# cinemere/evacuation

Hardware: AMD Instinct MI355X
Metric: env-steps/s (agent-updates/s) at n=60x4096 envs (higher is better)
Workload: dtype f32

## Files before the change

evacuation_amd/csrc/evac_api.hip:

```cpp
#include <hip/hip_runtime.h>

#include <cmath>
#include <cstddef>
#include <cstdio>
#include <cstdlib>
#include <cstring>
#include <mutex>
#include <new>
#include <string>
#include <vector>

#include "evac_device.h"
#include "evac_subwave.h"
#include "evac_team.h"
#include "evac_gather.h"
#include "evac_policy.h"
#include "evac_host.h"

namespace {

thread_local std::string g_create_error;

int validate(const evac_config_t* c, std::string& err) {
    if (!c) { err = "cfg is NULL"; return EVAC_ERR_INVALID_ARGUMENT; }
// ... 8 lines not shown
    if (c->type != EVAC_TYPE_DICT && c->type != EVAC_TYPE_BOX) { err = "type must be Dict|Box"; return EVAC_ERR_INVALID_ARGUMENT; }
    if (c->positions == EVAC_POS_GRAV && c->type == EVAC_TYPE_BOX) {
        err = "positions='grav' with type='Box' is not implemented (reference wrappers/config.py:79-80 raises NotImplementedError)";
        return EVAC_ERR_UNSUPPORTED;
    }
    return EVAC_OK;
}

int64_t obs_dim_of(const evac_config_t* c) {
    const int64_t n = c->number_of_pedestrians;
    if (c->positions == EVAC_POS_GRAV) return 6;
    const int64_t sc = c->statuses == EVAC_STAT_OHE ? 4 : (c->statuses == EVAC_STAT_CAT ? 1 : 0);
    if (c->type == EVAC_TYPE_BOX) return (n + 2) * (2 + sc);
    return 4 + 2 * n + sc * n;
}

}

enum class Form { Plain, Parts, Chain, Persist };

struct evac_handle {
    evac_config_t cfg;
    evac::Params p;
    int device;
    bool bound;
    int sub_lanes;
    bool cells;
    bool cu_wide;
    bool cu_wide4;
    bool default_cfg;
    int team_k;
    int32_t* sched;
    int sched_gen = -1;
    bool team_bound;
    int team_fit = -1;
    size_t team_xchg_bytes;
    bool team_coop;
    int cus;
    bool team_fault;
    volatile unsigned* team_flag_host;
    unsigned* team_flag_dev;
    std::string err;
    std::string variant[4];
    evac_options_t opt;
    Form form = Form::Plain;
    struct OwnStreams {
        hipStream_t s[2];
        hipEvent_t done[2], fork;
        bool pending;
        bool forked;
    } own;
    evac_handle* part[2];
    char* xchg;
    size_t xchg_bytes;
    unsigned* abort_word;
    hipEvent_t last_ev;
    struct ChainState {
        bool bound;
        bool small;
        bool restart = true;
        bool dirty;
        int gen = 1;
        int start = 1;
        int32_t* sched;
        unsigned long long wgs;
    } chain;
// ... 436 lines not shown
    __atomic_thread_fence(__ATOMIC_SEQ_CST);
    c->seq = (unsigned)h->persist.seq + 1u;
    __atomic_thread_fence(__ATOMIC_SEQ_CST);
    h->persist.seq += 1;
}
void release_own(evac_handle* h) {
    DeviceGuard g(h->device);
    for (int k = 0; k < 2; ++k)
        if (h->own.s[k]) (void)hipStreamSynchronize(h->own.s[k]);
    if (h->own.s[0] && h->own.s[1] && pools_on()) {
        std::lock_guard<std::mutex> lk(g_pool_mu);
        g_pool_pairs.push_back(PooledPair{h->device, {h->own.s[0], h->own.s[1]}});
        h->own.s[0] = h->own.s[1] = nullptr;
    }
    for (int k = 0; k < 2; ++k) {
        if (h->own.s[k]) (void)hipStreamDestroy(h->own.s[k]);
        if (h->own.done[k]) (void)hipEventDestroy(h->own.done[k]);
        if (h->part[k]) {
            give_error_word(h->device, (void*)h->part[k]->team_flag_host, (void*)h->part[k]->team_flag_dev);
            delete h->part[k];
        }
        h->part[k] = nullptr;
    }
    if (h->own.fork) (void)hipEventDestroy(h->own.fork);
    if (h->last_ev) (void)hipEventDestroy(h->last_ev);
    give_uncached(h->device, h->xchg, h->xchg_bytes);
    h->own = {};
    h->xchg = nullptr;
    h->xchg_bytes = 0;
    h->last_ev = nullptr;
    h->form = Form::Plain;
}
void deal_now(evac_handle_t h, hipStream_t s, bool both);
struct Deal { const int32_t* perm; int32_t* moving; const int32_t* loads; int32_t* next; };
Deal deal_of(const evac_handle* h, bool deals) {
    const int E = h->p.n_envs, g = h->sched_gen;
    const bool dealt = h->sched && g >= 0;
    deals = deals && dealt;
    return Deal{dealt ? h->sched + (2 + (g & 1)) * E : nullptr, h->sched ? h->sched + (dealt ? (g & 1) : 0) * E : nullptr,
                deals ? h->sched + ((g + 1) & 1) * E : nullptr, deals ? h->sched + (2 + ((g + 1) & 1)) * E : nullptr};
}
int launch_persistent(evac_handle* h, int resume, int stop_at, bool fresh) {
    using FW = evac::Wave<1, 1024>;
    using FW4 = evac::Wave<4, 1024>;
    hipStream_t S = h->own.s[0];
    const int E = h->p.n_envs;
    if (h->sched && h->sched_gen < 0) deal_now(h, S, true);
    const Deal d = deal_of(h, fresh);
    if (d.next) h->sched_gen += 1;
    evac::ChainArgs ca{h->xchg, h->persist.seq, nullptr, nullptr, 0, nullptr, resume, stop_at};
    if (h->team_k) {
        int32_t* decision = (int32_t*)(h->xchg + (size_t)evac::kPersistRing * 64 + 128) + E;
        if (hipMemsetAsync(h->p.team_rec, 0xff, h->team_xchg_bytes, S) != hipSuccess || hipMemsetAsync(decision, 0, 4 * (size_t)E, S) != hipSuccess) {
            (void)hipGetLastError();
            return fail(h, EVAC_ERR_HIP, "evac_rollout (persistent team kernel): hipMemsetAsync failed");
        }
        const int* np_ = nullptr;
        int* nq_ = nullptr;
        void* argv[] = {(void*)&h->p, (void*)&np_, (void*)&nq_, (void*)&np_, (void*)&nq_, (void*)&ca};
        const hipError_t le = launch_team_grid(h, team_persist_kernel(h), argv, S, true, false);
        if (le != hipSuccess) return fail(h, EVAC_ERR_HIP, std::string("evac_rollout (persistent team kernel): ") + hipGetErrorString(le));
    } else {
        const bool four = h->cu_wide4;
        const auto fn = four ? EVAC_PICK(h, k_rollout_persist_default_config, k_rollout_persist, FW4)
                             : EVAC_PICK(h, k_rollout_persist_default_config, k_rollout_persist, FW);
        const dim3 grid((unsigned)(E / (four ? FW4::kEnvsPerBlock : FW::kEnvsPerBlock)));
        hipLaunchKernelGGL(fn, grid, dim3(four ? FW4::kBlock : FW::kBlock), 0, S, h->p, d.perm, d.moving, d.loads, d.next, ca);
    }
    if (const int lc = check_launch(h, "evac_rollout (persistent kernel)"); lc != EVAC_OK) return lc;
    if (hipEventRecord(h->last_ev, S) != hipSuccess) { (void)hipGetLastError(); return fail(h, EVAC_ERR_HIP, "evac_rollout: event record behind the persistent kernel failed"); }
    return EVAC_OK;
}
int stop_persistent(evac_handle* h) {
    const int stop_index = h->persist.seq;
    post_command(h, 0, nullptr, nullptr, nullptr);
    h->persist.running = false;
    return launch_persistent(h, 1, stop_index, false);
}
int settle(evac_handle* h, hipStream_t stream, bool host_wait = false) {
    if (h->form == Form::Chain) h->chain.restart = true;
    if (!h->own.pending) return EVAC_OK;
// ... 152 lines not shown
    return EVAC_OK;
}

int64_t evac_obs_dim(evac_handle_t h) { return h ? h->p.obs_dim : -1; }
int32_t evac_num_envs(evac_handle_t h) { return h ? h->p.n_envs : -1; }

int64_t evac_algorithmic_bytes_per_env_step(evac_handle_t h) {
    if (!h) return -1;
    return 32ll * h->p.n_ped + 38ll + 4ll * h->p.obs_dim;
}

int evac_bind_state(evac_handle_t h, float* ped, uint8_t* status, float* agent, int32_t* clock, float* acc) {
    if (!h) return EVAC_ERR_INVALID_ARGUMENT;
    if (!ped || !status || !agent || !clock || !acc) return fail(h, EVAC_ERR_INVALID_ARGUMENT, "evac_bind_state: NULL buffer");
    if (((uintptr_t)ped | (uintptr_t)agent | (uintptr_t)clock | (uintptr_t)acc) & 15u)
        return fail(h, EVAC_ERR_INVALID_ARGUMENT, "evac_bind_state: ped/agent/clock/acc must be 16-byte aligned");
    if (const int rc = settle(h, nullptr, true); rc != EVAC_OK) return rc;
    h->p.ped = (float4*)ped;
    h->p.status = status;
    h->p.agent = (float4*)agent;
    h->p.clock = (int4*)clock;
    h->p.acc = (float4*)acc;
    h->bound = true;
    for (int k = 0; k < (h->form == Form::Parts ? 2 : 0); ++k) {
        const size_t first = (size_t)k * (size_t)h->part[k]->p.n_envs, N = (size_t)h->p.n_ped;
        const int rc = evac_bind_state(h->part[k], ped + first * N * 4, status + first * N, agent + first * 4, clock + first * 4, acc + first * 4);
        if (rc != EVAC_OK) return fail(h, rc, std::string("evac_bind_state (part): ") + h->part[k]->err);
    }
    return EVAC_OK;
}

namespace {
struct WorkspaceLayout {
    size_t sched, stats, team_rec, team_tile, team_xchg_end, chain_sched, chain_abort, total;
};
WorkspaceLayout workspace_layout(const evac_handle* h) {
    const size_t E = (size_t)h->p.n_envs;
    auto up = [](size_t x) { return (x + 255) & ~(size_t)255; };
    WorkspaceLayout w{};
    size_t o = 0;
    w.sched = o; o = up(o + 4 * E * sizeof(int32_t));
    w.stats = o; o = up(o + 64);
    if (h->form == Form::Chain) {
        w.chain_sched = o; o = up(o + 8 * E * sizeof(int32_t));
        w.chain_abort = o; o = up(o + 128);
    }
    if (h->team_k) {
        w.team_rec = o; o = up(o + evac::kTeamSets * E * 32 * 16);
        w.team_tile = o; o = up(o + evac::kTeamSets * E * 1024 * 16);
        w.team_xchg_end = o;
    }
    w.total = o;
    return w;
}
}

int64_t evac_workspace_bytes(evac_handle_t h) {
    if (!h) return -1;
    size_t total = workspace_layout(h).total, parts = 0;
    for (int k = 0; k < (h->form == Form::Parts ? 2 : 0); ++k) parts += workspace_layout(h->part[k]).total;
    return (int64_t)(parts > total ? parts : total);
}

int evac_bind_workspace(evac_handle_t h, void* workspace, int64_t bytes) {
    if (!h) return EVAC_ERR_INVALID_ARGUMENT;
    if (const int rc = settle(h, nullptr, true); rc != EVAC_OK) return rc;
    h->sched = nullptr;
    h->sched_gen = -1;
    h->team_bound = false;
    h->chain.bound = false;
    if (h->form == Form::Parts) {
        if (workspace && (bytes < evac_workspace_bytes(h) || ((uintptr_t)workspace & 255u)))
            return fail(h, EVAC_ERR_INVALID_ARGUMENT, "evac_bind_workspace: workspace smaller than evac_workspace_bytes() or not 256-byte aligned");
        size_t o = 0;
        for (int k = 0; k < 2; ++k) {
            const size_t t = workspace_layout(h->part[k]).total;
            const int rc = evac_bind_workspace(h->part[k], workspace ? (char*)workspace + o : nullptr, (int64_t)t);
            if (rc != EVAC_OK) return fail(h, rc, std::string("evac_bind_workspace (part): ") + h->part[k]->err);
            o += t;
        }
        return EVAC_OK;
    }
    if (!workspace) return EVAC_OK;
    const WorkspaceLayout w = workspace_layout(h);
    if (bytes < (int64_t)w.total) return fail(h, EVAC_ERR_INVALID_ARGUMENT, "evac_bind_workspace: workspace smaller than evac_workspace_bytes()");
    if ((uintptr_t)workspace & 255u) return fail(h, EVAC_ERR_INVALID_ARGUMENT, "evac_bind_workspace: workspace must be 256-byte aligned");
    char* base = (char*)workspace;
    h->sched = (int32_t*)(base + w.sched);
    if (h->form == Form::Chain) {
        h->chain.sched = (int32_t*)(base + w.chain_sched);
        h->abort_word = (unsigned*)(base + w.chain_abort);
        h->chain.dirty = false;
        h->chain.wgs = 0;
        h->chain.bound = true;
    }
    if (h->team_k) {
        h->p.team_err = h->team_flag_dev;
        h->p.team_rec = base + w.team_rec;
        h->p.team_tile = base + w.team_tile;
        h->team_xchg_bytes = w.team_xchg_end - w.team_rec;
        h->team_bound = true;
        DeviceGuard g(h->device);
        (void)team_grid_fits(h);
    }
    return EVAC_OK;
}

namespace {
void deal_now(evac_handle_t h, hipStream_t s, bool both) {
    const int E = h->p.n_envs;
    if (h->sched_gen < 0) h->sched_gen = 0;
    const int g = h->sched_gen;
    hipLaunchKernelGGL(evac::k_schedule, dim3(1), dim3(1024), 0, s, E, (const int*)(h->sched + ((g + 1) & 1) * E),
                       h->sched + (2 + (g & 1)) * E, both ? h->sched + (2 + ((g + 1) & 1)) * E : (int32_t*)nullptr,
                       h->cu_wide4 ? 4 : 16, h->cu_wide4 ? 4 : 1, 0);
}
}

int evac_reschedule(evac_handle_t h, void* stream) {
    if (!h) return EVAC_ERR_INVALID_ARGUMENT;
    if (const int rc = settle(h, (hipStream_t)stream); rc != EVAC_OK) return rc;
    if (h->form == Form::Chain) return EVAC_OK;
    if (h->form == Form::Parts) {
        for (int k = 0; k < 2; ++k)
            if (const int rc = evac_reschedule(h->part[k], stream); rc != EVAC_OK) return fail(h, rc, h->part[k]->err);
        return EVAC_OK;
    }
    if (!h->sched || !(h->cu_wide || h->cu_wide4)) return EVAC_OK;
    DeviceGuard g(h->device);
    deal_now(h, (hipStream_t)stream, true);
    return check_launch(h, "evac_reschedule");
}

int32_t evac_schedule_generation(evac_handle_t h) {
    if (h && h->form == Form::Parts) return evac_schedule_generation(h->part[0]);
    return (h && h->sched && (h->cu_wide || h->cu_wide4)) ? h->sched_gen : -1;
}

int evac_peer_gather(const float* src, int64_t rows, int32_t row_words, int32_t take_words, float* const* peer_dst, int32_t world,
                     int32_t my_rank, int32_t wgs_per_peer, void* stream) {
    if (!src || !peer_dst || rows <= 0 || row_words <= 0 || take_words <= 0 || take_words > row_words || world < 1 ||
        world > evac::kMaxPeers || my_rank < 0 || my_rank >= world)
        return EVAC_ERR_INVALID_ARGUMENT;
    if (rows * (int64_t)take_words >= (int64_t)1 << 31) return EVAC_ERR_INVALID_ARGUMENT;
    evac::PeerPtrs pp{};
    for (int r = 0; r < world; ++r) {
        if (!peer_dst[r]) return EVAC_ERR_INVALID_ARGUMENT;
        pp.dst[r] = peer_dst[r];
// ... 137 lines not shown
        h->persist.first = h->persist.seq;
    } else if (hipEventQuery(h->last_ev) == hipSuccess) {
        if (const int rc = launch_persistent(h, 1, 0x7fffffff, false); rc != EVAC_OK) return rc;
    } else {
        (void)hipGetLastError();
    }
    post_command(h, (int)n_steps, slab_out, final_stats, nullptr);
    h->own.pending = true;
    return EVAC_OK;
}

static int rollout_chain(evac_handle* h, int32_t n_steps, const float* actions, float* slab_out, evac_episode_stats_t* final_stats, hipStream_t s_) {
    using FW = evac::Wave<1, 1024>;
    using FW4 = evac::Wave<4, 1024>;
    using FS = evac::Wave<1, 256>;
    evac_handle::ChainState& ch = h->chain;
    const int wpe = h->cu_wide4 ? 4 : 1, per_wg = (h->cu_wide4 || ch.small) ? 4 : 16;
    const int E = h->p.n_envs, c = ch.gen;
    hipStream_t S = h->own.s[c & 1], O = h->own.s[(c + 1) & 1];
    const bool fork = ch.restart || !h->own.forked || actions != nullptr;
    if (fork) {
        if (hipEventRecord(h->own.fork, s_) != hipSuccess || hipStreamWaitEvent(S, h->own.fork, 0) != hipSuccess) {
            (void)hipGetLastError();
            return fail(h, EVAC_ERR_HIP, "evac_rollout: fork of the chain failed");
        }
        h->own.forked = true;
    }
    int32_t* moving = ch.sched;
    int32_t* perm = ch.sched + 4 * (size_t)E;
    if (ch.restart) {
        hipLaunchKernelGGL(evac::k_chain_import, dim3((unsigned)((E * wpe + 3) / 4)), dim3(256), 0, S, h->p, h->xchg, c, h->abort_word, ch.wgs, wpe);
        if (!ch.small) {
            hipLaunchKernelGGL(evac::k_schedule, dim3(1), dim3(1024), 0, S, E, (const int*)(moving + ((c + 3) & 3) * (size_t)E),
                               perm + (c & 3) * (size_t)E, (int32_t*)nullptr, per_wg, wpe == 4 ? 4 : 1, option_value("EVAC_CHAIN_DEAL", 0));
            hipLaunchKernelGGL(evac::k_copy_perm3, dim3(64), dim3(256), 0, S, E, (const int*)(perm + (c & 3) * (size_t)E),
                               perm + ((c + 1) & 3) * (size_t)E, perm + ((c + 2) & 3) * (size_t)E, perm + ((c + 3) & 3) * (size_t)E);
        }
        if (hipEventRecord(h->last_ev, S) != hipSuccess || hipStreamWaitEvent(O, h->last_ev, 0) != hipSuccess) {
            (void)hipGetLastError();
            return fail(h, EVAC_ERR_HIP, "evac_rollout: restart of the chain failed");
        }
        ch.start = c;
        ch.restart = false;
    }
    const bool deals = !ch.small && c - ch.start >= 2;
    const int32_t* deal_loads = deals ? moving + ((c + 2) & 3) * (size_t)E : nullptr;
    int32_t* deal_perm = deals ? perm + ((c + 2) & 3) * (size_t)E : nullptr;
    unsigned long long* started = (unsigned long long*)(h->abort_word + 8);
    if (ch.wgs > 0 && hipStreamWaitValue64(S, started, ch.wgs, hipStreamWaitValueGte, ~0ull) != hipSuccess) {
        (void)hipGetLastError();
        return fail(h, EVAC_ERR_HIP, "evac_rollout: hipStreamWaitValue64 (the chain's dispatch gate) failed");
    }
    static const int deal_mode = option_value("EVAC_CHAIN_DEAL", 0);
    evac::ChainArgs ca{h->xchg, c, h->abort_word, h->team_flag_dev, deal_mode, started};
    evac::Params pp = h->p;
    if (h->team_fault && c == ch.start + 1) pp.n_envs = E - per_wg;
    const auto fn = ch.small ? EVAC_PICK(h, k_rollout_chain_default_config, k_rollout_chain, FS)
                  : h->cu_wide4 ? EVAC_PICK(h, k_rollout_chain_default_config, k_rollout_chain, FW4)
                                : EVAC_PICK(h, k_rollout_chain_default_config, k_rollout_chain, FW);
    const dim3 grid((unsigned)(E / per_wg)), block(ch.small ? FS::kBlock : (h->cu_wide4 ? FW4::kBlock : FW::kBlock));
    hipLaunchKernelGGL(fn, grid, block, 0, S, pp, (int)n_steps, (const float2*)actions, slab_out, final_stats,
                       (const int*)(ch.small ? nullptr : perm + (c & 3) * (size_t)E), (int*)(ch.small ? nullptr : moving + (c & 3) * (size_t)E),
                       deal_loads, deal_perm, ca);
    if (const int lc = check_launch(h, "evac_rollout (chained)"); lc != EVAC_OK) return lc;
    ch.wgs += (unsigned long long)grid.x;
    ch.gen = c + 1;
    h->own.pending = true;
    ch.dirty = true;
    return EVAC_OK;
}

static int rollout_team(evac_handle* h, int32_t n_steps, const float* actions, float* slab_out, evac_episode_stats_t* final_stats, hipStream_t s_) {
    if (hipMemsetAsync(h->p.team_rec, 0xff, h->team_xchg_bytes, s_) != hipSuccess) return fail(h, EVAC_ERR_HIP, "evac_rollout: hipMemsetAsync failed");
    int n_steps_ = (int)n_steps;
    const float2* actions_ = (const float2*)actions;
    const int* perm_ = nullptr;
    int* moving_ = nullptr;
    void* argv[] = {(void*)&h->p, (void*)&n_steps_, (void*)&actions_, (void*)&slab_out, (void*)&final_stats, (void*)&perm_, (void*)&moving_,
                    (void*)&perm_, (void*)&moving_};
    const hipError_t le = launch_team_grid(h, team_kernel(h), argv, s_, !capturing(s_), h->team_coop);
    if (le != hipSuccess) return fail(h, EVAC_ERR_HIP, std::string("evac_rollout (team launch): ") + hipGetErrorString(le));
    return EVAC_OK;
}

static int rollout_plain(evac_handle* h, int32_t n_steps, const float* actions, float* actions_out, float* slab_out,
                         evac_episode_stats_t* final_stats, int32_t capture_envs, float* capture, const float* noise, hipStream_t stream) {
    if (capture || actions_out || noise) {
        EVAC_DISPATCH(h, k_rollout_diag, stream, h->p, (int)n_steps, (const float2*)actions, (float2*)actions_out, slab_out,
                      final_stats, (int)capture_envs, capture, noise);
    } else if (h->team_k && h->team_bound && team_grid_fits(h)) {
        return rollout_team(h, n_steps, actions, slab_out, final_stats, stream);
    } else if (h->cu_wide || h->cu_wide4) {
        using FW = evac::Wave<1, 1024>;
        using FW4 = evac::Wave<4, 1024>;
        const int E = h->p.n_envs;
        const bool cap = capturing(stream);
        const bool in_kernel = n_steps < 50 && E >= (h->cu_wide4 ? 4 : 16);
        if (h->sched && !cap && (h->sched_gen < 0 || !in_kernel)) deal_now(h, stream, h->sched_gen < 0);
        const Deal d = deal_of(h, !cap && in_kernel);
        if (h->sched && h->sched_gen >= 0 && !cap) h->sched_gen += 1;
        const bool four = h->cu_wide4;
        const auto fn = four ? EVAC_PICK(h, k_rollout_default_config, k_rollout, FW4) : EVAC_PICK(h, k_rollout_default_config, k_rollout, FW);
        const int per_block = four ? FW4::kEnvsPerBlock : FW::kEnvsPerBlock;
        hipLaunchKernelGGL(fn, dim3((unsigned)((E + per_block - 1) / per_block)), dim3(four ? FW4::kBlock : FW::kBlock), 0, stream,
                           h->p, (int)n_steps, (const float2*)actions, slab_out, final_stats, d.perm, d.moving, d.loads, d.next);
    } else if (h->default_cfg) {
        EVAC_DISPATCH(h, k_rollout_default_config, stream, h->p, (int)n_steps, (const float2*)actions, slab_out, final_stats,
                      (const int*)nullptr, (int*)nullptr, (const int*)nullptr, (int*)nullptr);
    } else {
        EVAC_DISPATCH(h, k_rollout, stream, h->p, (int)n_steps, (const float2*)actions, slab_out, final_stats, (const int*)nullptr,
                      (int*)nullptr, (const int*)nullptr, (int*)nullptr);
    }
    return check_launch(h, "evac_rollout");
}

int evac_rollout(evac_handle_t h, int32_t n_steps, const float* actions, float* actions_out, float* slab_out,
                 evac_episode_stats_t* final_stats, int32_t capture_envs, float* capture, const float* noise,
                 void* stream) {
    EVAC_REQUIRE_BOUND(h, "evac_rollout");
    if (n_steps < 1) return fail(h, EVAC_ERR_INVALID_ARGUMENT, "evac_rollout: n_steps must be >= 1");
    if (!slab_out) return fail(h, EVAC_ERR_INVALID_ARGUMENT, "evac_rollout: slab_out must be non-NULL");
    if (((uintptr_t)actions | (uintptr_t)actions_out) & 7u)
        return fail(h, EVAC_ERR_INVALID_ARGUMENT, "evac_rollout: actions buffers must be 8-byte aligned");
    DeviceGuard g(h->device);
    if (capture && (capture_envs < 1 || capture_envs > h->p.n_envs))
        return fail(h, EVAC_ERR_INVALID_ARGUMENT, "evac_rollout: capture_envs must be in [1, num_envs] when capture is given");
    hipStream_t s_ = (hipStream_t)stream;
    if (!(capture || actions_out || noise)) {
        if (h->form == Form::Parts) return rollout_parts(h, n_steps, actions, slab_out, final_stats, s_);
        if (h->form == Form::Persist && !actions && (!h->team_k || (h->team_bound && team_grid_fits(h))) && !capturing(s_))
            return rollout_persist(h, n_steps, slab_out, final_stats, s_);
        if (h->form == Form::Chain && h->chain.bound && !capturing(s_)) return rollout_chain(h, n_steps, actions, slab_out, final_stats, s_);
    }
    if (const int rc = settle(h, s_); rc != EVAC_OK) return rc;
    return rollout_plain(h, n_steps, actions, actions_out, slab_out, final_stats, capture_envs, capture, noise, s_);
}

int evac_observe(evac_handle_t h, float* obs_out, void* stream) {
    EVAC_REQUIRE_SETTLED(h, "evac_observe", stream);
    if (!obs_out) return fail(h, EVAC_ERR_INVALID_ARGUMENT, "evac_observe: obs_out is NULL");
    DeviceGuard g(h->device);
    EVAC_DISPATCH(h, k_observe, stream, h->p, obs_out);
    return check_launch(h, "evac_observe");
}
// ... 109 lines not shown
```

evacuation_amd/csrc/evac_device.h:

```cpp
#pragma once

#include <type_traits>

#include "evac_common.h"
#include "evac_families.h"


namespace evac {

template <class F>
__device__ __forceinline__ void grav_observation(const Params& p, typename F::Ctx& c, bool active, const Ped& q,
                                                 const Env& e, float (&o6)[6]) {
    Sums s{};
    float gx = 0.0f, gy = 0.0f;
    const bool visc = active && q.st == kViscek;
    grav_term(p, e.ax - q.x, e.ay - q.y, gx, gy);
    s.f0 = visc ? gx : 0.0f;
    s.f1 = visc ? gy : 0.0f;
    s.f2 = 0.0f;
    const unsigned long long pred[8] = {ballot(active && q.st == kFollower), 0, 0, 0, 0, 0, 0, 0};
    F::template reduce<true>(p, c, s, pred);
    float ex, ey;
    grav_term(p, e.ax - kExitX, e.ay - kExitY, ex, ey);
    const float nf = (float)s.i[0];
// ... 234 lines not shown
            b[k] = e < n_envs ? loads[e] : -1;
        }
#pragma unroll
        for (int k = 0; k < kPer; ++k)
            if (b[k] >= 0) atomicAdd(&hist[schedule_bin(b[k], unit)], 1);
    }
    __syncthreads();
    if (tid < kWave) {
        const int v = hist[tid];
        const int incl = wave_inclusive_scan(v);
        __builtin_amdgcn_fence(__ATOMIC_ACQ_REL, "wavefront");
        hist[tid] = incl - v;
        if (tid == kWave - 1) hist[kWave] = incl;
    }
    __syncthreads();
    for (int base = 0; base < n_envs; base += kPer * 1024) {
        int r[kPer];
#pragma unroll
        for (int k = 0; k < kPer; ++k) {
            const int e = base + k * 1024 + tid;
            r[k] = e < n_envs ? loads[e] : -1;
        }
#pragma unroll
        for (int k = 0; k < kPer; ++k)
            if (r[k] >= 0) r[k] = atomicAdd(&hist[schedule_bin(r[k], unit)], 1);
#pragma unroll
        for (int k = 0; k < kPer; ++k) {
            const int e = base + k * 1024 + tid;
            if (e < n_envs) perm[schedule_slot(r[k], n_envs, per_wg, mode)] = e;
        }
    }
}

__device__ __forceinline__ void pace_step(int* slot, const int* mine, int lane, int t, int& seen, int& prio) {
    *slot = t;
    const unsigned ahead_mask = (unsigned)ballot(seen >= t) & 0xfu;
    seen = mine[lane & 3];
    const int ahead = __popc(ahead_mask) & 3;
    if (ahead != prio) {
        prio = ahead;
        set_wave_priority(ahead);
    }
}


template <class F, bool GRAV, bool NORM>
__device__ __forceinline__ void step_outputs(const Params& p, typename F::Ctx& w, bool active, Ped& q, Env& e, StepOut& o,
                                             uint32_t gid, int autoreset, float* __restrict__ obs_out,
                                             float* __restrict__ reward_out, uint8_t* __restrict__ term_out,
                                             uint8_t* __restrict__ trunc_out, float* __restrict__ final_obs,
                                             evac_episode_stats_t* __restrict__ final_stats, const NormArgs& na) {
    const bool done = o.terminated || o.truncated;
    const int D = p.obs_dim;
    float* obs = obs_out + (size_t)w.env * D;
    float* fo = final_obs ? final_obs + (size_t)w.env * D : nullptr;
    double* ns = NORM ? na.state + (size_t)w.env * (3 * D + 4) : nullptr;
    float o6[6] = {e.ax, e.ay, o.ex, o.ey, o.gx, o.gy};
    float t6[6] = {o6[0], o6[1], o6[2], o6[3], o6[4], o6[5]};
    const bool reset_now = done && autoreset;
    if (reset_now) {
        if constexpr (!GRAV) {
            if (fo) {
                if constexpr (NORM) write_obs_generic(p, w.i, active, q, e, StoreNorm{fo, ns, D, na.eps, na.obs_clip});
                else write_obs_generic(p, w.i, active, q, e, StorePlain{fo});
            }
        }
// ... 107 lines not shown
EVAC_STEP_KERNEL(k_step_raw, false)
EVAC_STEP_KERNEL(k_step_norm, true)
#undef EVAC_STEP_KERNEL
#define EVAC_STEP_KERNEL_DEFAULT(NAME, NORM_)                                                                                  \
    template <class F, bool GRAV>                                                                                              \
    __global__ __launch_bounds__(F::kBlock, 4) void NAME(                                                                       \
        Params p, const float2* __restrict__ actions, const float* __restrict__ noise_in, float* __restrict__ obs_out,          \
        float* __restrict__ reward_out, uint8_t* __restrict__ term_out, uint8_t* __restrict__ trunc_out, int autoreset,         \
        float* __restrict__ final_obs, evac_episode_stats_t* __restrict__ final_stats, NormArgs na) {                           \
        __shared__ typename F::Smem sm;                                                                                         \
        const Params q = default_config_constants<GRAV>(p);                                                                     \
        step_kernel_body<F, GRAV, NORM_>(sm, q, actions, noise_in, obs_out, reward_out, term_out, trunc_out, autoreset, final_obs, \
                                         final_stats, na);                                                                      \
    }
EVAC_STEP_KERNEL_DEFAULT(k_step_default_config, false)
EVAC_STEP_KERNEL_DEFAULT(k_step_norm_default_config, true)
#undef EVAC_STEP_KERNEL_DEFAULT

__device__ __forceinline__ void capture_state(const Params& p, float* __restrict__ capture, int capture_envs, int t, int env, int i,
                                              bool active, bool owner, const Ped& q, const Env& e) {
    float* cp = capture + (((size_t)t * capture_envs + env) * (p.n_ped + 1)) * 3;
    if (active) {
        cp[3 * i + 0] = q.x;
        cp[3 * i + 1] = q.y;
        cp[3 * i + 2] = (float)q.st;
    }
    if (owner) {
        cp[3 * p.n_ped + 0] = e.ax;
        cp[3 * p.n_ped + 1] = e.ay;
        cp[3 * p.n_ped + 2] = 0.0f;
    }
}

template <class F, bool GRAV, bool DIAG, bool CHAIN = false, bool PERSIST = false>
__device__ __forceinline__ void rollout_body(
    typename F::Smem& sm, const Params& p, int n_steps, const float2* __restrict__ actions, float2* __restrict__ actions_out,
    float* __restrict__ slab_out, evac_episode_stats_t* __restrict__ final_stats, int capture_envs,
    float* __restrict__ capture, const float* __restrict__ noise_in, const int* __restrict__ perm = nullptr,
    int* __restrict__ moving_out = nullptr, const int* __restrict__ deal_loads = nullptr, int* __restrict__ deal_perm = nullptr,
    ChainArgs chain = ChainArgs{nullptr, 0, nullptr, nullptr}) {
    if constexpr (CHAIN) {
        if (threadIdx.x == 0) (void)__hip_atomic_fetch_add(chain.started, 1ull, __ATOMIC_RELAXED, __HIP_MEMORY_SCOPE_SYSTEM);
    }
    typename F::Ctx w(sm);
    if (w.env >= p.n_envs) return;
    const int my_slot = w.env;
    if (perm) w.env = __builtin_amdgcn_readfirstlane(perm[w.env]);
    F::init(w);
    const bool active = w.i < p.n_ped;
    Ped q;
    Env e;
    if constexpr (!CHAIN) load_env(p, w.env, w.i, active, q, e);
    if constexpr (F::kPace) {
        if (deal_perm && blockIdx.x == 0) {
            const int lightest = deal_loads[perm[0]];
            if (4 * lightest <= 3 * p.n_ped)
                schedule_envs_by_workgroup(sm.deal_hist, (int)threadIdx.x, p.n_envs, deal_loads, deal_perm, F::kEnvsPerBlock, F::WPE == 1 ? 1 : 4,
                                           CHAIN ? chain.deal_mode : 0);
        }
    }
    if constexpr (CHAIN) {
        static_assert(!F::kHelpers && (F::kPace || F::WPE == 1), "chained launches: one-wave envs (any workgroup size), and four-wave envs in CU-wide workgroups (a barrier per env)");
        constexpr int T = F::kThreadsPerEnv;
        if constexpr (F::WPE == 1) {
            if (!chain_wait<T>(chain, w.env)) {
                chain_give_up(chain, w.lane, w.env);
                return;
            }
            load_record<T>(chain.xchg + (size_t)w.env * Xchg<T>::kBytes, w.lane, w.lane, active, q, e);
        } else {
            if (w.wave_in_env == 0) {
                const bool ok = chain_wait<T>(chain, w.env);
                if (w.lane == 0) sm.chain_ok[w.slot] = ok ? 1 : 0;
            }
            F::sync(w);
            if (sm.chain_ok[w.slot] == 0) {
                if (w.wave_in_env == 0) chain_give_up(chain, w.lane, w.env);
                return;
            }
            load_record<T>(chain.xchg + (size_t)w.env * Xchg<T>::kBytes, w.i, w.lane, active, q, e);
        }
    }
    const uint32_t gid = p.env_id_offset + (uint32_t)w.env;
    const size_t E = (size_t)p.slab_envs;
    const int row = p.obs_dim + 3;
    uint32_t nzw[4] = {0u, 0u, 0u, 0u};
    int noise_group = -1;
// ... 152 lines not shown
                if (w.wave_in_env == 0) {
                    __builtin_amdgcn_fence(__ATOMIC_ACQ_REL, "wavefront");
                    if (fl_s <= t - stage_t0) {
                        const float v = sm.stage[w.slot][fl_s][fl_k];
                        float* dst = &slab_out[((size_t)(stage_t0 + fl_s) * E + w.env) * kGravRow + fl_k];
                        *dst = v;
                    }
                }
                stage_off = 0;
                stage_t0 = t + 1;
                flush_t = min(t + kStageSteps, n_steps - 1);
            }
        } else {
            bool stores = true;
            if constexpr (F::kHelpers) stores = !w.helper;
            if constexpr (F::kPipelined) stores = stores && o.done;
            if (stores) write_obs_generic(p, w.i, active, q, e, StorePlain{rowp});
            if (w.owner) {
                rowp[p.obs_dim + 0] = o.reward;
                rowp[p.obs_dim + 1] = f_term;
                rowp[p.obs_dim + 2] = f_trunc;
            }
        }
        if (slot64 == 63) {
            asm volatile("");
            if (t + 1 < n_steps) draw_actions(t + 1);
        }
    }
    if constexpr (!PERSIST) break;
    cmd_index += 1;
    t_base += n_steps;
    }
    if constexpr (F::kEnvBarrier) {
        if (moving_out && w.owner) moving_out[w.env] = w.have_next ? w.next_cols : p.n_ped;
    }
    if constexpr (F::kThreadsPerEnv == kWave) {
        if (moving_out) {
            const int nm = ballot(needs_row(p, q.st)) != 0ull ? wave_count((unsigned)(q.st - kViscek) < 3u) : 0;
            if (w.owner) moving_out[w.env] = nm;
        }
    }
    if constexpr (F::kHelpers) {
        if (F::aborted(w)) return;
    }
    if constexpr (CHAIN) {
        constexpr int T = F::kThreadsPerEnv;
        char* rec = chain.xchg + (size_t)w.env * Xchg<T>::kBytes;
        if constexpr (F::WPE == 1) {
            store_record<T>(rec, w.lane, w.lane, true, active, q, e);
            wait_vmem();
            if (w.lane == 0) store_dev_i32(rec + Xchg<T>::kGen, chain.gen + 1);
        } else {
            store_record<T>(rec, w.i, w.lane, w.wave_in_env == 0, active, q, e);
            wait_vmem();
            F::sync(w);
            if (w.wave_in_env == 0 && w.lane == 0) store_dev_i32(rec + Xchg<T>::kGen, chain.gen + 1);
        }
    } else {
        store_env(p, w.env, w.i, active, w.owner, q, e);
        if constexpr (PERSIST) {
            if (w.owner) store_dev_i32(persist_next_cmd(chain.xchg) + w.env, cmd_index);
        }
    }
}

template <class F, bool GRAV>
__global__ __launch_bounds__(F::kBlock, 4) void k_rollout(
    Params p, int n_steps, const float2* __restrict__ actions, float* __restrict__ slab_out,
    evac_episode_stats_t* __restrict__ final_stats, const int* __restrict__ perm, int* __restrict__ moving_out,
    const int* __restrict__ deal_loads, int* __restrict__ deal_perm) {
    __shared__ typename F::Smem sm;
    rollout_body<F, GRAV, false>(sm, p, n_steps, actions, nullptr, slab_out, final_stats, 0, nullptr, nullptr, perm, moving_out,
                                 deal_loads, deal_perm);
}

template <class F, bool GRAV>
__global__ __launch_bounds__(F::kBlock, 4) void k_rollout_default_config(
    Params p, int n_steps, const float2* __restrict__ actions, float* __restrict__ slab_out,
    evac_episode_stats_t* __restrict__ final_stats, const int* __restrict__ perm, int* __restrict__ moving_out,
    const int* __restrict__ deal_loads, int* __restrict__ deal_perm) {
    __shared__ typename F::Smem sm;
    const Params q = default_config_constants<GRAV>(p);
    rollout_body<F, GRAV, false>(sm, q, n_steps, actions, nullptr, slab_out, final_stats, 0, nullptr, nullptr, perm, moving_out,
                                 deal_loads, deal_perm);
}

template <class F, bool GRAV>
__global__ __launch_bounds__(F::kBlock, 4) void k_rollout_chain(
    Params p, int n_steps, const float2* __restrict__ actions, float* __restrict__ slab_out,
    evac_episode_stats_t* __restrict__ final_stats, const int* __restrict__ perm, int* __restrict__ moving_out,
    const int* __restrict__ deal_loads, int* __restrict__ deal_perm, ChainArgs chain) {
    __shared__ typename F::Smem sm;
    rollout_body<F, GRAV, false, true>(sm, p, n_steps, actions, nullptr, slab_out, final_stats, 0, nullptr, nullptr, perm, moving_out,
                                       deal_loads, deal_perm, chain);
}
template <class F, bool GRAV>
__global__ __launch_bounds__(F::kBlock, 4) void k_rollout_chain_default_config(
    Params p, int n_steps, const float2* __restrict__ actions, float* __restrict__ slab_out,
    evac_episode_stats_t* __restrict__ final_stats, const int* __restrict__ perm, int* __restrict__ moving_out,
    const int* __restrict__ deal_loads, int* __restrict__ deal_perm, ChainArgs chain) {
    __shared__ typename F::Smem sm;
    const Params q = default_config_constants<GRAV>(p);
    rollout_body<F, GRAV, false, true>(sm, q, n_steps, actions, nullptr, slab_out, final_stats, 0, nullptr, nullptr, perm, moving_out,
                                       deal_loads, deal_perm, chain);
}
template <class F, bool GRAV>
__global__ __launch_bounds__(F::kBlock, 4) void k_rollout_persist(
    Params p, const int* __restrict__ perm, int* __restrict__ moving_out, const int* __restrict__ deal_loads, int* __restrict__ deal_perm,
    ChainArgs chain) {
    __shared__ typename F::Smem sm;
    rollout_body<F, GRAV, false, false, true>(sm, p, 0, nullptr, nullptr, nullptr, nullptr, 0, nullptr, nullptr, perm, moving_out,
                                              deal_loads, deal_perm, chain);
}
template <class F, bool GRAV>
__global__ __launch_bounds__(F::kBlock, 4) void k_rollout_persist_default_config(
    Params p, const int* __restrict__ perm, int* __restrict__ moving_out, const int* __restrict__ deal_loads, int* __restrict__ deal_perm,
    ChainArgs chain) {
// ... 14 lines not shown
    Ped q;
    Env e;
    load_env(p, env, idx, active, q, e);
    char* rec = xchg + (size_t)env * xchg_bytes(T);
    const int kXchgStatus = 16 * T, kXchgEnv = 20 * T, kXchgGen = 20 * T + 128;
    *(f4*)(rec + idx * 16) = active ? f4{q.x, q.y, q.dx, q.dy} : f4{0.0f, 0.0f, 0.0f, 0.0f};
    *(int*)(rec + kXchgStatus + idx * 4) = active ? q.st : 0;
    if (idx == 0) {
        *(f4*)(rec + kXchgEnv) = f4{e.ax, e.ay, e.adx, e.ady};
        *(f4*)(rec + kXchgEnv + 16) = f4{__builtin_bit_cast(float, e.now), __builtin_bit_cast(float, e.n_resets), __builtin_bit_cast(float, (int)e.total), 0.0f};
        *(f4*)(rec + kXchgEnv + 32) = f4{e.acc_ret, e.acc_intr, e.acc_stat, 0.0f};
        *(int*)(rec + kXchgGen) = gen;
    }
}
__global__ __launch_bounds__(256) void k_chain_export(Params p, const char* __restrict__ xchg, int wpe) {
    const int wv = blockIdx.x * 4 + (threadIdx.x >> 6), env = wv / wpe, part = wv - env * wpe, lane = threadIdx.x & 63;
    if (env >= p.n_envs) return;
    const int idx = part * 64 + lane;
    const bool active = idx < p.n_ped;
    Ped q;
    Env e;
    if (wpe == 1) load_record<64>(xchg + (size_t)env * Xchg<64>::kBytes, idx, lane, active, q, e);
    else load_record<256>(xchg + (size_t)env * Xchg<256>::kBytes, idx, lane, active, q, e);
    store_env(p, env, idx, active, idx == 0, q, e);
}
__global__ void k_copy_perm3(int n_envs, const int* __restrict__ src, int* __restrict__ a, int* __restrict__ b, int* __restrict__ c) {
    for (int e = blockIdx.x * blockDim.x + threadIdx.x; e < n_envs; e += gridDim.x * blockDim.x) {
        const int v = src[e];
        a[e] = v; b[e] = v; c[e] = v;
    }
}

__global__ __launch_bounds__(1024) void k_schedule(int n_envs, const int* __restrict__ moving, int* __restrict__ perm, int* __restrict__ perm_other,
                                                   int per_wg, int unit, int mode = 0) {
    __shared__ int hist[kWave + 2];
    schedule_envs_by_workgroup(hist, (int)threadIdx.x, n_envs, moving, perm, per_wg, unit, mode);
    if (perm_other) {
        __syncthreads();
        for (int e = threadIdx.x; e < n_envs; e += 1024) perm_other[e] = perm[e];
    }
}
template <class F, bool GRAV>
__global__ __launch_bounds__(F::kBlock, 4) void k_rollout_diag(
    Params p, int n_steps, const float2* __restrict__ actions, float2* __restrict__ actions_out,
    float* __restrict__ slab_out, evac_episode_stats_t* __restrict__ final_stats, int capture_envs,
    float* __restrict__ capture, const float* __restrict__ noise_in) {
    __shared__ typename F::Smem sm;
    rollout_body<F, GRAV, true>(sm, p, n_steps, actions, actions_out, slab_out, final_stats, capture_envs, capture, noise_in);
}

template <class F, bool GRAV>
__global__ __launch_bounds__(F::kBlock, 4) void k_reset(Params p, const uint8_t* __restrict__ mask,
                                                      const float4* __restrict__ draws, float* __restrict__ obs_out) {
    __shared__ typename F::Smem sm;
    typename F::Ctx w(sm);
    if (w.env >= p.n_envs) return;
    if (mask && !mask[w.env]) return;
    const bool active = w.i < p.n_ped;
    Ped q;
    Env e;
    load_env(p, w.env, w.i, active, q, e);
    const uint32_t gid = p.env_id_offset + (uint32_t)w.env;
    float4 d = make_float4(0.f, 0.f, 1.f, 0.f);
    if (active) d = draws ? draws[(size_t)w.env * p.n_ped + w.i] : philox_reset_draw(p, gid, w.i, e.n_resets);
    reset_env(p, active, d, q, e);
    if (obs_out) write_obs<F, GRAV>(p, w, active, true, q, e, obs_out + (size_t)w.env * p.obs_dim);
    store_env(p, w.env, w.i, active, w.owner, q, e);
}
// ... 113 lines not shown
```

evacuation_amd/csrc/evac_subwave.h:

```cpp
#pragma once

#include "evac_device.h"

namespace evac {

template <int G, bool GRAV>
__device__ __forceinline__ void autoreset_sub(const Params& p, typename Sub<G>::Ctx& w, bool active, bool done, uint32_t gid,
                                              Ped& q, Env& e, StepOut& o, float (&o6)[6], evac_episode_stats_t* stats_row) {
    finish_counts<Sub<G>>(p, w, q, o);
    if (done && stats_row && w.owner) write_stats(stats_row, e, o);
    Ped nq = q;
    Env ne = e;
    reset_env(p, active, philox_reset_draw(p, gid, w.i, e.n_resets), nq, ne);
    float n6[6] = {ne.ax, ne.ay, 0.f, 0.f, 0.f, 0.f};
    if constexpr (GRAV) grav_observation<Sub<G>>(p, w, active, nq, ne, n6);
    if (done) {
        q = nq;
        e = ne;
#pragma unroll
        for (int k = 0; k < 6; ++k) o6[k] = n6[k];
    }
}

template <int G, bool GRAV, bool NORM>
// ... 152 lines not shown
            if (noise_in) nz = active ? noise_in[((size_t)t * E + w.env) * p.n_ped + w.i] : 0.0f;
        }
        StepOut o;
        step_env<F, GRAV>(p, w, active, q, e, adir, nz, o);
        if (DIAG && capture && valid && w.env < capture_envs) capture_state(p, capture, capture_envs, t, w.env, w.i, active, w.owner, q, e);
        float o6[6] = {e.ax, e.ay, o.ex, o.ey, o.gx, o.gy};
        const bool done = o.terminated || o.truncated;
        if (ballot(done) != 0ull)
            autoreset_sub<G, GRAV>(p, w, active, done, gid, q, e, o, o6,
                                   (final_stats && valid) ? final_stats + (size_t)t * E + w.env : nullptr);
        if (valid) {
            float* rowp = slab_out + ((size_t)t * E + w.env) * row;
            if constexpr (GRAV) {
                if (owner) {
#pragma unroll
                    for (int k = 0; k < 6; ++k) rowp[k] = o6[k];
                }
            } else {
                write_obs_generic(p, w.i, active, q, e, StorePlain{rowp});
            }
            if (owner) {
                rowp[p.obs_dim + 0] = o.reward;
                rowp[p.obs_dim + 1] = o.terminated ? 1.0f : 0.0f;
                rowp[p.obs_dim + 2] = o.truncated ? 1.0f : 0.0f;
            }
        }
    }
    store_env(p, w.env, w.i, valid && active, owner, q, e);
}

template <int G, bool GRAV>
__global__ __launch_bounds__(256) void k_rollout_sub(Params p, int n_steps, const float2* __restrict__ actions,
                                                     float* __restrict__ slab_out,
                                                     evac_episode_stats_t* __restrict__ final_stats, const int*, int*, const int*, int*) {
    __shared__ typename Sub<G>::Smem sm;
    rollout_body_sub<G, GRAV, false>(sm, p, n_steps, actions, nullptr, slab_out, final_stats, 0, nullptr, nullptr);
}
template <int G, bool GRAV>
__global__ __launch_bounds__(256) void k_rollout_default_config_sub(Params p, int n_steps, const float2* __restrict__ actions,
                                                                    float* __restrict__ slab_out,
                                                                    evac_episode_stats_t* __restrict__ final_stats, const int*, int*, const int*, int*) {
    __shared__ typename Sub<G>::Smem sm;
    const Params q = default_config_constants<GRAV>(p);
    rollout_body_sub<G, GRAV, false>(sm, q, n_steps, actions, nullptr, slab_out, final_stats, 0, nullptr, nullptr);
}
template <int G, bool GRAV>
__global__ __launch_bounds__(256) void k_rollout_diag_sub(Params p, int n_steps, const float2* __restrict__ actions,
                                                          float2* __restrict__ actions_out, float* __restrict__ slab_out,
                                                          evac_episode_stats_t* __restrict__ final_stats,
                                                          int capture_envs, float* __restrict__ capture,
                                                          const float* __restrict__ noise_in) {
    __shared__ typename Sub<G>::Smem sm;
    rollout_body_sub<G, GRAV, true>(sm, p, n_steps, actions, actions_out, slab_out, final_stats, capture_envs, capture, noise_in);
}

template <int G, bool GRAV>
__global__ __launch_bounds__(256) void k_reset_sub(Params p, const uint8_t* __restrict__ mask, const float4* __restrict__ draws,
                                                   float* __restrict__ obs_out) {
    using F = Sub<G>;
    __shared__ typename F::Smem sm;
    typename F::Ctx w(sm);
    bool valid = w.env < p.n_envs;
    if (!valid) w.env = p.n_envs - 1;
    if (mask && !mask[w.env]) valid = false;
    const bool active = w.i < p.n_ped;
    Ped q;
    Env e;
    load_env(p, w.env, w.i, active, q, e);
    const uint32_t gid = p.env_id_offset + (uint32_t)w.env;
    float4 d = make_float4(0.f, 0.f, 1.f, 0.f);
    if (active) d = draws ? draws[(size_t)w.env * p.n_ped + w.i] : philox_reset_draw(p, gid, w.i, e.n_resets);
    reset_env(p, active, d, q, e);
    if (obs_out) write_obs<F, GRAV>(p, w, active, valid, q, e, obs_out + (size_t)w.env * p.obs_dim);
    store_env(p, w.env, w.i, valid && active, valid && w.owner, q, e);
// ... 18 lines not shown
```

Before: 691.7 million.

## Compute next-launch env schedule in last-finishing workgroup via ticket counter

```diff
diff --git a/evacuation_amd/csrc/evac_api.hip b/evacuation_amd/csrc/evac_api.hip
--- a/evacuation_amd/csrc/evac_api.hip
+++ b/evacuation_amd/csrc/evac_api.hip
@@ -64,6 +64,7 @@
     int team_k;
     int32_t* sched;
     int sched_gen = -1;
+    unsigned* deal_ticket;
     bool team_bound;
     int team_fit = -1;
     size_t team_xchg_bytes;
@@ -566,13 +567,15 @@
     h->form = Form::Plain;
 }
 void deal_now(evac_handle_t h, hipStream_t s, bool both);
-struct Deal { const int32_t* perm; int32_t* moving; const int32_t* loads; int32_t* next; };
-Deal deal_of(const evac_handle* h, bool deals) {
+enum { kDealNone = 0, kDealFront = 1, kDealTail = 2 };
+struct Deal { const int32_t* perm; int32_t* moving; const int32_t* loads; int32_t* next; unsigned* ticket; };
+Deal deal_of(const evac_handle* h, int deals) {
     const int E = h->p.n_envs, g = h->sched_gen;
     const bool dealt = h->sched && g >= 0;
-    deals = deals && dealt;
+    if (!dealt) deals = kDealNone;
     return Deal{dealt ? h->sched + (2 + (g & 1)) * E : nullptr, h->sched ? h->sched + (dealt ? (g & 1) : 0) * E : nullptr,
-                deals ? h->sched + ((g + 1) & 1) * E : nullptr, deals ? h->sched + (2 + ((g + 1) & 1)) * E : nullptr};
+                deals ? h->sched + ((g + (deals == kDealTail ? 0 : 1)) & 1) * E : nullptr, deals ? h->sched + (2 + ((g + 1) & 1)) * E : nullptr,
+                deals == kDealTail ? h->deal_ticket : nullptr};
 }
 int launch_persistent(evac_handle* h, int resume, int stop_at, bool fresh) {
     using FW = evac::Wave<1, 1024>;
@@ -580,7 +583,7 @@
     hipStream_t S = h->own.s[0];
     const int E = h->p.n_envs;
     if (h->sched && h->sched_gen < 0) deal_now(h, S, true);
-    const Deal d = deal_of(h, fresh);
+    const Deal d = deal_of(h, fresh ? kDealFront : kDealNone);
     if (d.next) h->sched_gen += 1;
     evac::ChainArgs ca{h->xchg, h->persist.seq, nullptr, nullptr, 0, nullptr, resume, stop_at};
     if (h->team_k) {
@@ -799,7 +802,7 @@
 
 namespace {
 struct WorkspaceLayout {
-    size_t sched, stats, team_rec, team_tile, team_xchg_end, chain_sched, chain_abort, total;
+    size_t sched, ticket, team_rec, team_tile, team_xchg_end, chain_sched, chain_abort, total;
 };
 WorkspaceLayout workspace_layout(const evac_handle* h) {
     const size_t E = (size_t)h->p.n_envs;
@@ -807,7 +810,7 @@
     WorkspaceLayout w{};
     size_t o = 0;
     w.sched = o; o = up(o + 4 * E * sizeof(int32_t));
-    w.stats = o; o = up(o + 64);
+    w.ticket = o; o = up(o + 64);
     if (h->form == Form::Chain) {
         w.chain_sched = o; o = up(o + 8 * E * sizeof(int32_t));
         w.chain_abort = o; o = up(o + 128);
@@ -834,6 +837,7 @@
     if (const int rc = settle(h, nullptr, true); rc != EVAC_OK) return rc;
     h->sched = nullptr;
     h->sched_gen = -1;
+    h->deal_ticket = nullptr;
     h->team_bound = false;
     h->chain.bound = false;
     if (h->form == Form::Parts) {
@@ -854,6 +858,7 @@
     if ((uintptr_t)workspace & 255u) return fail(h, EVAC_ERR_INVALID_ARGUMENT, "evac_bind_workspace: workspace must be 256-byte aligned");
     char* base = (char*)workspace;
     h->sched = (int32_t*)(base + w.sched);
+    h->deal_ticket = (unsigned*)(base + w.ticket);
     if (h->form == Form::Chain) {
         h->chain.sched = (int32_t*)(base + w.chain_sched);
         h->abort_word = (unsigned*)(base + w.chain_abort);
@@ -880,7 +885,7 @@
     const int g = h->sched_gen;
     hipLaunchKernelGGL(evac::k_schedule, dim3(1), dim3(1024), 0, s, E, (const int*)(h->sched + ((g + 1) & 1) * E),
                        h->sched + (2 + (g & 1)) * E, both ? h->sched + (2 + ((g + 1) & 1)) * E : (int32_t*)nullptr,
-                       h->cu_wide4 ? 4 : 16, h->cu_wide4 ? 4 : 1, 0);
+                       h->cu_wide4 ? 4 : 16, h->cu_wide4 ? 4 : 1, 0, h->deal_ticket);
 }
 }
 
@@ -1084,7 +1089,7 @@
         hipLaunchKernelGGL(evac::k_chain_import, dim3((unsigned)((E * wpe + 3) / 4)), dim3(256), 0, S, h->p, h->xchg, c, h->abort_word, ch.wgs, wpe);
         if (!ch.small) {
             hipLaunchKernelGGL(evac::k_schedule, dim3(1), dim3(1024), 0, S, E, (const int*)(moving + ((c + 3) & 3) * (size_t)E),
-                               perm + (c & 3) * (size_t)E, (int32_t*)nullptr, per_wg, wpe == 4 ? 4 : 1, option_value("EVAC_CHAIN_DEAL", 0));
+                               perm + (c & 3) * (size_t)E, (int32_t*)nullptr, per_wg, wpe == 4 ? 4 : 1, option_value("EVAC_CHAIN_DEAL", 0), (unsigned*)nullptr);
             hipLaunchKernelGGL(evac::k_copy_perm3, dim3(64), dim3(256), 0, S, E, (const int*)(perm + (c & 3) * (size_t)E),
                                perm + ((c + 1) & 3) * (size_t)E, perm + ((c + 2) & 3) * (size_t)E, perm + ((c + 3) & 3) * (size_t)E);
         }
@@ -1128,8 +1133,9 @@
     const float2* actions_ = (const float2*)actions;
     const int* perm_ = nullptr;
     int* moving_ = nullptr;
+    unsigned* ticket_ = nullptr;
     void* argv[] = {(void*)&h->p, (void*)&n_steps_, (void*)&actions_, (void*)&slab_out, (void*)&final_stats, (void*)&perm_, (void*)&moving_,
-                    (void*)&perm_, (void*)&moving_};
+                    (void*)&perm_, (void*)&moving_, (void*)&ticket_};
     const hipError_t le = launch_team_grid(h, team_kernel(h), argv, s_, !capturing(s_), h->team_coop);
     if (le != hipSuccess) return fail(h, EVAC_ERR_HIP, std::string("evac_rollout (team launch): ") + hipGetErrorString(le));
     return EVAC_OK;
@@ -1147,21 +1153,26 @@
         using FW4 = evac::Wave<4, 1024>;
         const int E = h->p.n_envs;
         const bool cap = capturing(stream);
-        const bool in_kernel = n_steps < 50 && E >= (h->cu_wide4 ? 4 : 16);
-        if (h->sched && !cap && (h->sched_gen < 0 || !in_kernel)) deal_now(h, stream, h->sched_gen < 0);
-        const Deal d = deal_of(h, !cap && in_kernel);
+        static const int deal_opt = option_value("EVAC_PLAIN_DEAL", 0);
+        const int per_wg = h->cu_wide4 ? 4 : 16;
+        const bool can_front = E >= per_wg;
+        const bool can_tail = E % per_wg == 0 && E <= evac::kTailDealMaxEnvs && (!h->cu_wide4 || h->default_cfg);
+        int deal = deal_opt == 1 ? kDealNone : deal_opt == 2 ? kDealFront : deal_opt == 3 ? kDealTail : (n_steps < 100 ? kDealFront : kDealTail);
+        if ((deal == kDealFront && !can_front) || (deal == kDealTail && !can_tail) || cap) deal = kDealNone;
+        if (h->sched && !cap && (h->sched_gen < 0 || deal == kDealNone)) deal_now(h, stream, h->sched_gen < 0);
+        const Deal d = deal_of(h, deal);
         if (h->sched && h->sched_gen >= 0 && !cap) h->sched_gen += 1;
         const bool four = h->cu_wide4;
         const auto fn = four ? EVAC_PICK(h, k_rollout_default_config, k_rollout, FW4) : EVAC_PICK(h, k_rollout_default_config, k_rollout, FW);
         const int per_block = four ? FW4::kEnvsPerBlock : FW::kEnvsPerBlock;
         hipLaunchKernelGGL(fn, dim3((unsigned)((E + per_block - 1) / per_block)), dim3(four ? FW4::kBlock : FW::kBlock), 0, stream,
-                           h->p, (int)n_steps, (const float2*)actions, slab_out, final_stats, d.perm, d.moving, d.loads, d.next);
+                           h->p, (int)n_steps, (const float2*)actions, slab_out, final_stats, d.perm, d.moving, d.loads, d.next, d.ticket);
     } else if (h->default_cfg) {
         EVAC_DISPATCH(h, k_rollout_default_config, stream, h->p, (int)n_steps, (const float2*)actions, slab_out, final_stats,
-                      (const int*)nullptr, (int*)nullptr, (const int*)nullptr, (int*)nullptr);
+                      (const int*)nullptr, (int*)nullptr, (const int*)nullptr, (int*)nullptr, (unsigned*)nullptr);
     } else {
         EVAC_DISPATCH(h, k_rollout, stream, h->p, (int)n_steps, (const float2*)actions, slab_out, final_stats, (const int*)nullptr,
-                      (int*)nullptr, (const int*)nullptr, (int*)nullptr);
+                      (int*)nullptr, (const int*)nullptr, (int*)nullptr, (unsigned*)nullptr);
     }
     return check_launch(h, "evac_rollout");
 }
diff --git a/evacuation_amd/csrc/evac_device.h b/evacuation_amd/csrc/evac_device.h
--- a/evacuation_amd/csrc/evac_device.h
+++ b/evacuation_amd/csrc/evac_device.h
@@ -290,6 +290,52 @@
     }
 }
 
+constexpr int kTailDealMaxEnvs = 16 * 1024;
+__device__ __forceinline__ void tail_deal(int* hist, int n_envs, const int* loads, int* __restrict__ perm, unsigned* ticket, int per_wg, int unit) {
+    constexpr int kPer = kTailDealMaxEnvs / 1024;
+    const int tid = (int)threadIdx.x;
+    int* last = &hist[kWave + 1];
+    wait_vmem();
+    __syncthreads();
+    if (tid == 0) {
+        const unsigned t = __hip_atomic_fetch_add(ticket, 1u, __ATOMIC_RELAXED, __HIP_MEMORY_SCOPE_AGENT);
+        const bool is_last = (int)(t + 1u) * per_wg >= n_envs;
+        if (is_last) __hip_atomic_store(ticket, 0u, __ATOMIC_RELAXED, __HIP_MEMORY_SCOPE_AGENT);
+        *last = is_last ? 1 : 0;
+    }
+    __syncthreads();
+    if (*last == 0) return;
+    int b[kPer];
+#pragma unroll
+    for (int k = 0; k < kPer; ++k) {
+        b[k] = 0;
+        if (k * 1024 < n_envs) b[k] = __hip_atomic_load(loads + min(k * 1024 + tid, n_envs - 1), __ATOMIC_RELAXED, __HIP_MEMORY_SCOPE_AGENT);
+    }
+    if (tid <= kWave) hist[tid] = 0;
+    __syncthreads();
+#pragma unroll
+    for (int k = 0; k < kPer; ++k) {
+        b[k] = k * 1024 + tid < n_envs ? schedule_bin(b[k], unit) : -1;
+        if (b[k] >= 0) atomicAdd(&hist[b[k]], 1);
+    }
+    __syncthreads();
+    if (tid < kWave) {
+        const int v = hist[tid];
+        const int incl = wave_inclusive_scan(v);
+        __builtin_amdgcn_fence(__ATOMIC_ACQ_REL, "wavefront");
+        hist[tid] = incl - v;
+        if (tid == kWave - 1) hist[kWave] = incl;
+    }
+    __syncthreads();
+#pragma unroll
+    for (int k = 0; k < kPer; ++k) {
+        if (b[k] >= 0) {
+            const int r = atomicAdd(&hist[b[k]], 1);
+            perm[schedule_slot(r, n_envs, per_wg)] = k * 1024 + tid;
+        }
+    }
+}
+
 __device__ __forceinline__ void pace_step(int* slot, const int* mine, int lane, int t, int& seen, int& prio) {
     *slot = t;
     const unsigned ahead_mask = (unsigned)ballot(seen >= t) & 0xfu;
@@ -463,13 +509,14 @@
     }
 }
 
-template <class F, bool GRAV, bool DIAG, bool CHAIN = false, bool PERSIST = false>
+template <class F, bool GRAV, bool DIAG, bool CHAIN = false, bool PERSIST = false, bool TAIL = false>
 __device__ __forceinline__ void rollout_body(
     typename F::Smem& sm, const Params& p, int n_steps, const float2* __restrict__ actions, float2* __restrict__ actions_out,
     float* __restrict__ slab_out, evac_episode_stats_t* __restrict__ final_stats, int capture_envs,
     float* __restrict__ capture, const float* __restrict__ noise_in, const int* __restrict__ perm = nullptr,
     int* __restrict__ moving_out = nullptr, const int* __restrict__ deal_loads = nullptr, int* __restrict__ deal_perm = nullptr,
-    ChainArgs chain = ChainArgs{nullptr, 0, nullptr, nullptr}) {
+    ChainArgs chain = ChainArgs{nullptr, 0, nullptr, nullptr}, unsigned* deal_ticket = nullptr) {
+    static_assert(!TAIL || (F::kPace && !DIAG && !CHAIN && !PERSIST), "the tail deal: plain launches of the CU-wide families");
     if constexpr (CHAIN) {
         if (threadIdx.x == 0) (void)__hip_atomic_fetch_add(chain.started, 1ull, __ATOMIC_RELAXED, __HIP_MEMORY_SCOPE_SYSTEM);
     }
@@ -483,7 +530,9 @@
     Env e;
     if constexpr (!CHAIN) load_env(p, w.env, w.i, active, q, e);
     if constexpr (F::kPace) {
-        if (deal_perm && blockIdx.x == 0) {
+        bool front = deal_perm && blockIdx.x == 0;
+        if constexpr (TAIL) front = front && !deal_ticket;
+        if (front) {
             const int lightest = deal_loads[perm[0]];
             if (4 * lightest <= 3 * p.n_ped)
                 schedule_envs_by_workgroup(sm.deal_hist, (int)threadIdx.x, p.n_envs, deal_loads, deal_perm, F::kEnvsPerBlock, F::WPE == 1 ? 1 : 4,
@@ -702,12 +751,20 @@
     t_base += n_steps;
     }
     if constexpr (F::kEnvBarrier) {
-        if (moving_out && w.owner) moving_out[w.env] = w.have_next ? w.next_cols : p.n_ped;
+        if (moving_out && w.owner) {
+            const int nm = w.have_next ? w.next_cols : p.n_ped;
+            if constexpr (TAIL) __hip_atomic_store(moving_out + w.env, nm, __ATOMIC_RELAXED, __HIP_MEMORY_SCOPE_AGENT);
+            else moving_out[w.env] = nm;
+        }
     }
     if constexpr (F::kThreadsPerEnv == kWave) {
         if (moving_out) {
             const int nm = ballot(needs_row(p, q.st)) != 0ull ? wave_count((unsigned)(q.st - kViscek) < 3u) : 0;
-            if (w.owner) moving_out[w.env] = nm;
+            if constexpr (TAIL) {
+                if (w.owner) __hip_atomic_store(moving_out + w.env, nm, __ATOMIC_RELAXED, __HIP_MEMORY_SCOPE_AGENT);
+            } else {
+                if (w.owner) moving_out[w.env] = nm;
+            }
         }
     }
     if constexpr (F::kHelpers) {
@@ -731,6 +788,9 @@
         if constexpr (PERSIST) {
             if (w.owner) store_dev_i32(persist_next_cmd(chain.xchg) + w.env, cmd_index);
         }
+        if constexpr (TAIL) {
+            if (deal_ticket) tail_deal(sm.deal_hist, p.n_envs, moving_out, deal_perm, deal_ticket, F::kEnvsPerBlock, F::WPE == 1 ? 1 : 4);
+        }
     }
 }
 
@@ -738,21 +798,21 @@
 __global__ __launch_bounds__(F::kBlock, 4) void k_rollout(
     Params p, int n_steps, const float2* __restrict__ actions, float* __restrict__ slab_out,
     evac_episode_stats_t* __restrict__ final_stats, const int* __restrict__ perm, int* __restrict__ moving_out,
-    const int* __restrict__ deal_loads, int* __restrict__ deal_perm) {
+    const int* __restrict__ deal_loads, int* __restrict__ deal_perm, unsigned* deal_ticket) {
     __shared__ typename F::Smem sm;
-    rollout_body<F, GRAV, false>(sm, p, n_steps, actions, nullptr, slab_out, final_stats, 0, nullptr, nullptr, perm, moving_out,
-                                 deal_loads, deal_perm);
+    rollout_body<F, GRAV, false, false, false, F::kPace && F::WPE == 1>(sm, p, n_steps, actions, nullptr, slab_out, final_stats, 0, nullptr, nullptr, perm,
+                                                         moving_out, deal_loads, deal_perm, ChainArgs{nullptr, 0, nullptr, nullptr}, deal_ticket);
 }
 
 template <class F, bool GRAV>
 __global__ __launch_bounds__(F::kBlock, 4) void k_rollout_default_config(
     Params p, int n_steps, const float2* __restrict__ actions, float* __restrict__ slab_out,
     evac_episode_stats_t* __restrict__ final_stats, const int* __restrict__ perm, int* __restrict__ moving_out,
-    const int* __restrict__ deal_loads, int* __restrict__ deal_perm) {
+    const int* __restrict__ deal_loads, int* __restrict__ deal_perm, unsigned* deal_ticket) {
     __shared__ typename F::Smem sm;
     const Params q = default_config_constants<GRAV>(p);
-    rollout_body<F, GRAV, false>(sm, q, n_steps, actions, nullptr, slab_out, final_stats, 0, nullptr, nullptr, perm, moving_out,
-                                 deal_loads, deal_perm);
+    rollout_body<F, GRAV, false, false, false, F::kPace>(sm, q, n_steps, actions, nullptr, slab_out, final_stats, 0, nullptr, nullptr, perm,
+                                                         moving_out, deal_loads, deal_perm, ChainArgs{nullptr, 0, nullptr, nullptr}, deal_ticket);
 }
 
 template <class F, bool GRAV>
@@ -833,8 +893,9 @@
 }
 
 __global__ __launch_bounds__(1024) void k_schedule(int n_envs, const int* __restrict__ moving, int* __restrict__ perm, int* __restrict__ perm_other,
-                                                   int per_wg, int unit, int mode = 0) {
+                                                   int per_wg, int unit, int mode = 0, unsigned* ticket = nullptr) {
     __shared__ int hist[kWave + 2];
+    if (ticket && threadIdx.x == 0) *ticket = 0u;
     schedule_envs_by_workgroup(hist, (int)threadIdx.x, n_envs, moving, perm, per_wg, unit, mode);
     if (perm_other) {
         __syncthreads();
diff --git a/evacuation_amd/csrc/evac_subwave.h b/evacuation_amd/csrc/evac_subwave.h
--- a/evacuation_amd/csrc/evac_subwave.h
+++ b/evacuation_amd/csrc/evac_subwave.h
@@ -208,14 +208,14 @@
 template <int G, bool GRAV>
 __global__ __launch_bounds__(256) void k_rollout_sub(Params p, int n_steps, const float2* __restrict__ actions,
                                                      float* __restrict__ slab_out,
-                                                     evac_episode_stats_t* __restrict__ final_stats, const int*, int*, const int*, int*) {
+                                                     evac_episode_stats_t* __restrict__ final_stats, const int*, int*, const int*, int*, unsigned*) {
     __shared__ typename Sub<G>::Smem sm;
     rollout_body_sub<G, GRAV, false>(sm, p, n_steps, actions, nullptr, slab_out, final_stats, 0, nullptr, nullptr);
 }
 template <int G, bool GRAV>
 __global__ __launch_bounds__(256) void k_rollout_default_config_sub(Params p, int n_steps, const float2* __restrict__ actions,
                                                                     float* __restrict__ slab_out,
-                                                                    evac_episode_stats_t* __restrict__ final_stats, const int*, int*, const int*, int*) {
+                                                                    evac_episode_stats_t* __restrict__ final_stats, const int*, int*, const int*, int*, unsigned*) {
     __shared__ typename Sub<G>::Smem sm;
     const Params q = default_config_constants<GRAV>(p);
     rollout_body_sub<G, GRAV, false>(sm, q, n_steps, actions, nullptr, slab_out, final_stats, 0, nullptr, nullptr);
```

New measurement: 669.7 million. 3.2% lower.
